# duxfrederic/lightcurver

Measured on AMD Instinct MI355X. Metric: cutouts/sec (PSF-fit + joint forward-model iter), 32x32 & 64x64 stamps, higher is better.
Workload: dtype f32

## Files before the change

### lightcurver_amd/csrc/psf_kernels.h

```cpp
#pragma once
#include <type_traits>
#include <utility>

#include "lc_common.h"
#include "starlet_device.h"

#ifndef LC_XPOLL_SLEEP
#define LC_XPOLL_SLEEP 2
#endif
#ifndef LC_P5_AHEAD
#define LC_P5_AHEAD 1
#endif
#ifndef LC_STARLET_LIVE_ADDR
#define LC_STARLET_LIVE_ADDR 1
#endif
#ifndef LC_SERIAL_TRIM
#define LC_SERIAL_TRIM 1
#endif
namespace lc {
constexpr int kXFlagStride = 16;

#ifdef LC_STAMPS
__device__ long long g_stamps[128];
#define LC_STAMP(k)                                                      \
  do {                                                                   \
    if ((blockIdx.x == 0 || blockIdx.x == 8) && threadIdx.x == 0 && it == A.n_iter - 1)  \
      g_stamps[(k) + (blockIdx.x == 8 ? 64 : 0)] = clock64();            \
  } while (0)
#else
#define LC_STAMP(k) do {} while (0)
#endif


struct PsfArgs {
  int F, S, n_iter, t0, hist_stride, mode;
  const float *data, *wgt;
  const float *W;
  const float *norms;
  const float *Tm;
  float *B, *mB, *sB;
  float *stars, *stars_m, *stars_s;
  float *hist;
  float *qscratch;
  float *out_loss, *out_chi2, *out_gstars, *out_ggrid, *out_gT, *out_model;
  float lam_sc, lam_hf;
  lc_adabelief_cfg ab;
  float *xch;
  int *xflags, *xabort;
  int launch_seq, heal, force_abort_it;
  const float *bkB, *bkmB, *bksB, *bkstars, *bkstars_m, *bkstars_s;
  int *heal_count;
  const float *ext_grad;
  const float *sched;
  float *B1, *mB1, *sB1;
  int xcd_fast;
};

typedef float lc_v4f __attribute__((ext_vector_type(4)));
__device__ __forceinline__ void store_sc1_x4(float *p, lc_v4f v) {
  asm volatile("global_store_dwordx4 %0, %1, off sc1\n\ts_nop 2" ::"v"(p), "v"(v) : "memory");
}
__device__ __forceinline__ void store_plain_x4(float *p, lc_v4f v) {
  asm volatile("global_store_dwordx4 %0, %1, off\n\ts_nop 2" ::"v"(p), "v"(v) : "memory");
}
__device__ __forceinline__ void store_sc1_f(float *p, float v) {
  asm volatile("global_store_dword %0, %1, off sc1" ::"v"(p), "v"(v) : "memory");
}
__device__ __forceinline__ void load_sc1_2x4(const float *p, lc_v4f &a, lc_v4f &b) {
  asm volatile("global_load_dwordx4 %0, %2, off sc1\n\tglobal_load_dwordx4 %1, %2, off offset:16 sc1\n\ts_waitcnt vmcnt(0)"
               : "=&v"(a), "=&v"(b)
               : "v"(p)
               : "memory");
}
__device__ __forceinline__ void load_sc1_2x4_1(const float *p, lc_v4f &a, lc_v4f &b, const float *ps, float &s) {
  asm volatile("global_load_dword %2, %4, off sc1\n\tglobal_load_dwordx4 %0, %3, off sc1\n\tglobal_load_dwordx4 %1, %3, off offset:16 sc1\n\ts_waitcnt vmcnt(0)"
               : "=&v"(a), "=&v"(b), "=&v"(s)
               : "v"(p), "v"(ps)
               : "memory");
}
__device__ __forceinline__ void load_sc1_x4(const float *p, lc_v4f &a) {
  asm volatile("global_load_dwordx4 %0, %1, off sc1\n\ts_waitcnt vmcnt(0)" : "=&v"(a) : "v"(p) : "memory");
}
__device__ __forceinline__ float load_sc1_f(const float *p) {
  float v;
  asm volatile("global_load_dword %0, %1, off sc1\n\ts_waitcnt vmcnt(0)" : "=&v"(v) : "v"(p) : "memory");
  return v;
}


template <int N_, int SS_, int PX_, int SG_, bool WC_ = false, int JB_ = 8>
struct PsfCfg {
  static constexpr int N = N_, SS = SS_, PX = PX_, SG = SG_;
  static constexpr bool WC = WC_;
  static constexpr int n = N / SS;
  static constexpr int NTHR = N * N / PX;
  static constexpr int NW = (NTHR + kWave - 1) / kWave;
  static constexpr int NT = ntaps(SS);
  static constexpr int J = ilog2(N);
  static constexpr int LR = 8;
  static constexpr int LC = (JB_ * (N_ / SS_) / 4 >= 64) ? 4 : 2;
  static constexpr int LA = LC;
  static constexpr int TS = N + 1;
  static constexpr int RS = n + 1;
  static constexpr int OFF_T = 0;
  static constexpr int SZ_T = WC_ ? N * (N + 2 * (N / 4 + 10) + 1) : N * TS;
  static constexpr int OFF_R = OFF_T + SZ_T;
  static constexpr int SZ_R2 = SG * n * TS;
  static constexpr int VS = WC_ ? n + 3 : RS, VO = WC_ ? 1 : 0;
  static constexpr int SZ_V = SG * N * VS;
  static constexpr int JB = JB_;
  static constexpr int AP = N / 4 + 10;
  static constexpr int TSA = N + 2 * AP + 1;
  static constexpr int APR = AP / SS + 2;
  static constexpr int JBP = JB + 1;
  static constexpr int WSZ = JB * TSA + (n + 2 * APR) * JBP;
  static constexpr int SZ_VR = (SZ_V > StarletLds<N>::FLOATS) ? SZ_V : StarletLds<N>::FLOATS;
  static constexpr int OFF_WSC = OFF_R + SZ_VR;
  static constexpr int SZ_R = WC ? (SZ_VR + NW * WSZ) : ((2 * SZ_R2 > SZ_V) ? 2 * SZ_R2 : SZ_V);
  static constexpr int OFF_RES = OFF_R + SZ_R;
  static constexpr int SZ_RES = WC ? 0 : SG * n * n;
  static constexpr int OFF_TAPS = OFF_RES + SZ_RES;
  static constexpr int NTP = NT + 3;
  static constexpr int SZ_TAPS = (16 * 4 * NTP + 1) / 2 * 2 + 16 * 2 * NT * 2;
  static constexpr int OFF_TAPP = OFF_TAPS + (16 * 4 * NTP + 1) / 2 * 2;
  static constexpr int OFF_RED = OFF_TAPS + SZ_TAPS;
  static constexpr int IPS = n * n / LC;
  static constexpr int IPS_PAD = (IPS + kWave - 1) / kWave * kWave;
  static constexpr int SLOTS = IPS_PAD / kWave;
  static constexpr int SZ_REDX = 16 * NW;
  static constexpr int SZ_RED = (WC ? 16 * (n / JB) * 5 : SG * SLOTS * 5) + SZ_REDX + NW + 8;
  static constexpr int OFF_REDX = OFF_RED + (WC ? 16 * (n / JB) * 5 : SG * SLOTS * 5);
  static constexpr int OFF_REDW = OFF_REDX + SZ_REDX;
  static constexpr int OFF_STAR = OFF_RED + SZ_RED;
  static constexpr int MAXS = 16;
  static constexpr int SZ_STAR = MAXS * 20 + 16;
  static constexpr int LDS_FLOATS = OFF_STAR + SZ_STAR;
  static_assert(WC || StarletLds<N>::FLOATS <= SZ_T + SZ_R + SZ_RES, "starlet ping-pong buffers must fit over T + R + RES");
  static_assert(PX % SS == 0 && N % PX == 0 && n % LR == 0 && n % LC == 0 && n % LA == 0 && n % JB == 0, "tiling");
  static_assert(LDS_FLOATS * 4 <= 163840, "LDS");
  static_assert(OFF_TAPP % 2 == 0, "tap pairs are read as 64-bit words");
  static_assert(NTHR <= 1024 && NTHR % kWave == 0, "threads");
  static_assert(!WC_ || PX_ <= 8, "the WC layout keeps the pixel state in registers");
};


template <int SS, int NT>
__device__ inline void tap_entry(float delta, int k, float &tap, float &dtap, int &bq) {
  const int o = (int)nearbyintf(delta);
  const int base = o - kRg - (SS - 1);
  int q = base / SS;
  if (q * SS > base) --q;
  bq = q;
  const int m = q * SS + k;
  const float inv_s2 = 1.0f / (kSigmaG * kSigmaG);
  const float nrm = 0.3989422804014327f / kSigmaG;
  float a = 0.f, d = 0.f;
#pragma unroll
  for (int dv = 0; dv < SS; ++dv) {
    const int t = m + dv;
    if (t >= o - kRg && t <= o + kRg) {
      const float x = (float)t - delta;
      const float p = nrm * expf(-0.5f * x * x * inv_s2);
      a += p;
      d += p * x * inv_s2;
    }
  }
  tap = a;
  dtap = d;
}

template <class C, bool SPLIT = false>
__global__ __launch_bounds__(C::NTHR) void psf_fit_kernel(PsfArgs A) {
  constexpr int N = C::N, SS = C::SS, PX = C::PX, SG = C::SG, n = C::n, NT = C::NT, J = C::J;
  constexpr int NTHR = C::NTHR, TS = C::TS, RS = C::RS, LR = C::LR, LC = C::LC, LA = C::LA;
  extern __shared__ __align__(16) float lds[];
  float *T = lds + C::OFF_T;
  float *R2t = lds + C::OFF_R;
  float *R2xt = R2t + C::SZ_R2;
  float *V = lds + C::OFF_R;
  float *RES = lds + C::OFF_RES;
  float *TAPS = lds + C::OFF_TAPS + 1;
  constexpr int NTP = C::NTP;
  lc_v2f *TAPP = (lc_v2f *)(lds + C::OFF_TAPP);
  float *REDX = lds + C::OFF_REDX;
  float *RED = lds + C::OFF_RED;
  float *REDW = lds + C::OFF_REDW;
  float *SCAL = REDW + C::NW;
  float *SP = lds + C::OFF_STAR;
  float *SGR = SP + C::MAXS * 4;
  float *SM = SGR + C::MAXS * 5;
  float *SV = SM + C::MAXS * 4;
  int *BQ = (int *)(SV + C::MAXS * 4);

  int f = blockIdx.x, role = 0;
  if constexpr (SPLIT) {
    f = ((int)blockIdx.x >> 4) * 8 + ((int)blockIdx.x & 7);
    role = ((int)blockIdx.x >> 3) & 1;
    if (f >= A.F) return;
  }
  const bool conv_role = !SPLIT || role == 0, starlet_role = !SPLIT || role == 1;
  const int my_xcc = SPLIT ? (int)(__builtin_amdgcn_s_getreg(20 | (3 << 11)) & 15u) : 0;
  int same_xcd = 0;
  const int tid0 = threadIdx.x;
  const int S = A.S;

  const float *dataf = A.data + (size_t)f * S * n * n;
  const float *wgtf = A.wgt + (size_t)f * S * n * n;

  if constexpr (!SPLIT) {
    if (A.heal) {
      if (__hip_atomic_load(A.xabort, __ATOMIC_RELAXED, __HIP_MEMORY_SCOPE_AGENT) != A.launch_seq) return;
      const size_t o = (size_t)f * N * N;
      for (int i = tid0; i < N * N; i += NTHR) {
        A.B[o + i] = A.bkB[o + i];
        A.mB[o + i] = A.bkmB[o + i];
        A.sB[o + i] = A.bksB[o + i];
      }
      if (tid0 < S * 4) {
        A.stars[(size_t)f * S * 4 + tid0] = A.bkstars[(size_t)f * S * 4 + tid0];
        A.stars_m[(size_t)f * S * 4 + tid0] = A.bkstars_m[(size_t)f * S * 4 + tid0];
        A.stars_s[(size_t)f * S * 4 + tid0] = A.bkstars_s[(size_t)f * S * 4 + tid0];
      }
      if (f == 0 && tid0 == 0) atomicAdd(A.heal_count, 1);
      __threadfence_block();
      __syncthreads();
    }
  }

  if constexpr (C::WC) {
    for (int i = tid0; i < C::SZ_T; i += NTHR) lds[C::OFF_T + i] = 0.f;
    for (int i = tid0; i < C::NW * C::WSZ; i += NTHR) lds[C::OFF_WSC + i] = 0.f;
  }
  if (tid0 < S * 4) {
    SP[tid0] = A.stars[(size_t)f * S * 4 + tid0];
    SM[tid0] = A.stars_m[(size_t)f * S * 4 + tid0];
    SV[tid0] = A.stars_s[(size_t)f * S * 4 + tid0];
  }
  __syncthreads();

  constexpr bool STATE_REGS = (PX <= 8);
  float *Bg = A.B, *mBg = A.mB, *sBg = A.sB;
  if constexpr (SPLIT && !STATE_REGS) {
    if (role == 1) {
      const size_t g0pix = (size_t)f * N * N + (size_t)(tid0 / (N / PX)) * N + (tid0 % (N / PX)) * PX;
#pragma unroll
      for (int q = 0; q < PX / 4; ++q) {
        ((float4 *)(A.B1 + g0pix))[q] = ((const float4 *)(A.B + g0pix))[q];
        ((float4 *)(A.mB1 + g0pix))[q] = ((const float4 *)(A.mB + g0pix))[q];
        ((float4 *)(A.sB1 + g0pix))[q] = ((const float4 *)(A.sB + g0pix))[q];
      }
      Bg = A.B1;
      mBg = A.mB1;
      sBg = A.sB1;
    }
  }
  float Bp[PX], Mp[PX], Sp_[PX], Tp[PX];
  {
    const size_t g0pix = (size_t)f * N * N + (size_t)(tid0 / (N / PX)) * N + (tid0 % (N / PX)) * PX;
#pragma unroll
    for (int q = 0; q < PX / 4; ++q) {
      if (STATE_REGS) {
        const float4 b = ((const float4 *)(A.B + g0pix))[q], t = ((const float4 *)(A.Tm + g0pix))[q];
        const float4 m = ((const float4 *)(A.mB + g0pix))[q], sv = ((const float4 *)(A.sB + g0pix))[q];
        Bp[4 * q] = b.x; Bp[4 * q + 1] = b.y; Bp[4 * q + 2] = b.z; Bp[4 * q + 3] = b.w;
        Tp[4 * q] = t.x; Tp[4 * q + 1] = t.y; Tp[4 * q + 2] = t.z; Tp[4 * q + 3] = t.w;
        Mp[4 * q] = m.x; Mp[4 * q + 1] = m.y; Mp[4 * q + 2] = m.z; Mp[4 * q + 3] = m.w;
        Sp_[4 * q] = sv.x; Sp_[4 * q + 1] = sv.y; Sp_[4 * q + 2] = sv.z; Sp_[4 * q + 3] = sv.w;
      }
    }
  }

  auto compute_taps = [&](int tid) {
    for (int e = tid; e < S * 2 * NTP; e += NTHR) {
      const int s = e / (2 * NTP), ax = (e / NTP) & 1, k = e % NTP - 1;
      float tap = 0.f, dtap = 0.f;
      int bq = 0;
      const float c_off = (N % 2 == 0) ? 0.5f : 0.0f;
      const float delta = fminf(fmaxf(SS * SP[s * 4 + 1 + ax], -(float)(N / 4)), (float)(N / 4)) + c_off;
      if (k >= 0 && k < NT) tap_entry<SS, NT>(delta, k, tap, dtap, bq);
      TAPS[(s * 4 + 2 * ax) * NTP + k] = tap;
      TAPS[(s * 4 + 2 * ax + 1) * NTP + k] = dtap;
      if (k >= 0 && k < NT) TAPP[(s * 2 + ax) * NT + k] = (lc_v2f){tap, dtap};
      if (k == 0) BQ[s * 2 + ax] = bq;
    }
  };
  auto step_stars = [&](int tid) {
#pragma clang fp contract(off)
    if (tid < S * 3) {
      const float lr = SCAL[0], bc1 = SCAL[1], bc2 = SCAL[2];
      const float b1 = A.ab.b1, b2 = A.ab.b2, eps = A.ab.eps, eps_root = A.ab.eps_root;
      const int s = tid / 3, q = tid % 3;
      const float g = SGR[s * 5 + 1 + q];
      const float mn = b1 * SM[s * 4 + q] + (1.f - b1) * g;
      const float dg = g - mn;
      const float sn = b2 * SV[s * 4 + q] + (1.f - b2) * dg * dg + eps_root;
      SM[s * 4 + q] = mn;
      SV[s * 4 + q] = sn;
      SP[s * 4 + q] -= lr * (mn * bc1) / (sqrtf(sn * bc2) + eps);
    }
  };
  auto update_stars_and_taps = [&](int tid) {
    step_stars(tid);
    __syncthreads();
    compute_taps(tid);
  };
  if (conv_role) compute_taps(tid0);
  constexpr bool TRIM = SPLIT && C::WC && PX == 8 && LC_SERIAL_TRIM;
  static_assert(!TRIM || 3 * C::MAXS <= kWave, "the x0 sums and the stars' step are lanes of one wave");
  [[maybe_unused]] float tpix_next[TRIM ? PX : 1];
  if constexpr (TRIM) {
    if (role == 0) {
      const int pu = tid0 / (N / PX), pv = (tid0 % (N / PX)) * PX;
#pragma unroll
      for (int p = 0; p < PX; ++p) {
        tpix_next[p] = Bp[p] + Tp[p];
        T[pu * C::TSA + C::AP + pv + p] = tpix_next[p];
      }
    }
    __syncthreads();
  }
  for (int it = 0; it < A.n_iter; ++it) {
    const int tglob = A.t0 + it;
    if constexpr (SPLIT) {
      if (A.force_abort_it == it && f == 0 && role == 1) {
        if (tid0 == 0) __hip_atomic_store(A.xabort, A.launch_seq, __ATOMIC_RELAXED, __HIP_MEMORY_SCOPE_AGENT);
        break;
      }
    }
    int tid = tid0;
    LC_LAUNDER(tid);
    const int lane = tid & 63, wid = tid >> 6;
    const int pu = tid / (N / PX);
    const int pv = (tid % (N / PX)) * PX;
    const size_t gpix = (size_t)f * N * N + (size_t)pu * N + pv;
    if (tid < 3 && A.mode == 1) SCAL[tid] = A.sched[3 * tglob + tid];
    LC_STAMP(0);
    float gB[PX];
#pragma unroll
    for (int p = 0; p < PX; ++p) gB[p] = 0.f;
    float tpix[PX];
    if (conv_role) {
    if constexpr (TRIM) {
#pragma unroll
      for (int p = 0; p < PX; ++p) tpix[p] = tpix_next[p];
    } else if (C::WC && STATE_REGS) {
#pragma unroll
      for (int p = 0; p < PX; ++p) {
        tpix[p] = Bp[p] + Tp[p];
        T[pu * C::TSA + C::AP + pv + p] = tpix[p];
      }
    } else if (STATE_REGS) {
#pragma unroll
      for (int p = 0; p < PX; ++p) T[pu * TS + pv + p] = Bp[p] + Tp[p];
    } else {
      const float4 *bp = (const float4 *)(Bg + gpix);
      const float4 *tp = (const float4 *)(A.Tm + gpix);
#pragma unroll
      for (int q = 0; q < PX / 4; ++q) {
        const float4 b = bp[q], t = tp[q];
        T[pu * TS + pv + 4 * q + 0] = b.x + t.x;
        T[pu * TS + pv + 4 * q + 1] = b.y + t.y;
        T[pu * TS + pv + 4 * q + 2] = b.z + t.z;
        T[pu * TS + pv + 4 * q + 3] = b.w + t.w;
      }
    }
    if (tid < S * 5) SGR[tid] = 0.f;

    for (int g0 = 0; g0 < S; g0 += SG) {
      if (!TRIM || g0 > 0) __syncthreads();
      LC_STAMP(1 + 5 * (g0 / SG));
      if constexpr (C::WC) {
        constexpr int JB = C::JB, NBLK = n / JB;
        float *wsc = lds + C::OFF_WSC + wid * C::WSZ;
        constexpr int TSA = C::TSA, AP = C::AP, APR = C::APR;
        float *R2w = wsc + AP, *RESw = wsc + JB * TSA + APR * C::JBP;
        int kdone = 0;
        for (int task = wid; task < SG * NBLK; task += C::NW, ++kdone) {
          progress_prio(kdone);
          const int sl = task / NBLK, blk = task % NBLK, s = g0 + sl;
          if (s >= S) continue;
          const int jd0 = blk * JB;
          const float *tx = TAPS + (s * 4 + 0) * NTP, *ty = tx + 2 * NTP, *dty = tx + 3 * NTP;
          const int bqx = BQ[s * 2 + 0], bqy = BQ[s * 2 + 1];
          const float amp = SP[s * 4 + 0], sky = SP[s * 4 + 3];
          constexpr int NI3 = (JB * (n / LC) + 63) / 64;
          float dpre[NI3][LC], wpre[NI3][LC];
#pragma unroll
          for (int i3 = 0; i3 < NI3; ++i3) {
            const int item = lane + 64 * i3;
            const bool ok = item < JB * (n / LC);
            const int jl = item % JB, a0 = (item / JB) * LC;
#pragma unroll
            for (int j = 0; j < LC; ++j) {
              const size_t pix = ok ? ((size_t)s * n * n + (size_t)(a0 + j) * n + jd0 + jl) : 0;
              const float dv = dataf[pix], wv = wgtf[pix];
              dpre[i3][j] = ok ? dv : 0.f;
              wpre[i3][j] = ok ? wv : 0.f;
            }
          }
          LC_STAMP(10);
          {
            const int ws = SS * (jd0 - bqx) - (NT - 1);
            if constexpr (SS == 2) {
              constexpr int NP = (NT + 1) / 2, WL2 = (JB - 1) + NP;
              lc_v2f tr2[NP];
#pragma unroll
              for (int h = 0; h < NP; ++h) tr2[h] = (lc_v2f){tx[NT - 1 - 2 * h], tx[NT - 2 - 2 * h]};
              for (int u = lane; u < N; u += 64) {
                lc_v2f win2[WL2];
                const float *trow = T + u * TSA + AP + ws;
#pragma unroll
                for (int i = 0; i < WL2; ++i) win2[i] = (lc_v2f){trow[2 * i], trow[2 * i + 1]};
                lc_v2f acc[JB];
#pragma unroll
                for (int j = 0; j < JB; ++j) acc[j] = (lc_v2f){0.f, 0.f};
#pragma unroll
                for (int h = 0; h < NP; ++h) {
#pragma unroll
                  for (int j = 0; j < JB; ++j) acc[j] = pk_fma(tr2[h], win2[j + h], acc[j]);
                }
#pragma unroll
                for (int j = 0; j < JB; ++j) R2w[j * TSA + u] = acc[j].x + acc[j].y;
              }
            } else {
              constexpr int WL = SS * (JB - 1) + NT;
              float tk[NT];
#pragma unroll
              for (int k = 0; k < NT; ++k) tk[k] = tx[k];
              for (int u = lane; u < N; u += 64) {
                float win[WL];
                const float *trow = T + u * TSA + AP + ws;
#pragma unroll
                for (int i = 0; i < WL; ++i) win[i] = trow[i];
#pragma unroll
                for (int j = 0; j < JB; ++j) {
                  float acc = 0.f;
#pragma unroll
                  for (int k = 0; k < NT; ++k) acc = fmaf(tk[k], win[SS * j - k + NT - 1], acc);
                  R2w[j * TSA + u] = acc;
                }
              }
            }
          }
          wave_lds_sync();
          LC_STAMP(11);
          float chi = 0.f, ga = 0.f, gy = 0.f, gs = 0.f;
          {
            constexpr int WL = SS * (LC - 1) + NT;
            lc_v2f tyd[NT];
#pragma unroll
            for (int k = 0; k < NT; ++k) tyd[k] = TAPP[(s * 2 + 1) * NT + k];
#pragma unroll
            for (int i3 = 0; i3 < NI3; ++i3) {
              const int item = lane + 64 * i3;
              if (item < JB * (n / LC)) {
                const int jl = item % JB, a0 = (item / JB) * LC;
                const int ws = SS * (a0 - bqy) - (NT - 1);
                float win[WL];
                const float *r2 = R2w + jl * TSA + ws;
#pragma unroll
                for (int i = 0; i < WL; ++i) win[i] = r2[i];
                float lgy = 0.f;
                lc_v2f fvys[LC];
#pragma unroll
                for (int j = 0; j < LC; ++j) fvys[j] = (lc_v2f){0.f, 0.f};
#pragma unroll
                for (int k = 0; k < NT; ++k) {
#pragma unroll
                  for (int j = 0; j < LC; ++j) fvys[j] = pk_fma(tyd[k], pk_bcast(win[SS * j - k + NT - 1]), fvys[j]);
                  if constexpr (LC == 4) asm volatile("" : "+v"(fvys[0]), "+v"(fvys[1]), "+v"(fvys[2]), "+v"(fvys[3]));
                  else asm volatile("" : "+v"(fvys[0]), "+v"(fvys[1]));
                }
#pragma unroll
                for (int j = 0; j < LC; ++j) {
                  const float fv = fvys[j].x, fy = fvys[j].y;
                  const float model = fmaf(amp, fv, sky);
                  const float res = model - dpre[i3][j];
                  const float rw = wpre[i3][j] * res;
                  chi = fmaf(rw, res, chi);
                  ga = fmaf(rw, fv, ga);
                  lgy = fmaf(rw, fy, lgy);
                  gs += rw;
                  RESw[(a0 + j) * C::JBP + jl] = rw;
                  if (A.out_model) A.out_model[(size_t)f * S * n * n + (size_t)s * n * n + (size_t)(a0 + j) * n + jd0 + jl] = model;
                }
                gy += lgy * amp * SS;
              }
            }
          }
          wave_sum4(chi, ga, gy, gs);
          if (lane == 0) {
            float *r = RED + (s * NBLK + blk) * 5;
            r[0] = chi;
            r[1] = ga;
            r[3] = gy;
            r[4] = gs;
          }
          wave_lds_sync();
          LC_STAMP(12);
          {
            constexpr int WI = (SS * LA - 1 + NT - 1) / SS + 1;
            constexpr int NI4 = (JB * (n / LA) + 63) / 64;
            if constexpr (SS == 2) {
              constexpr int NP = (NT + 1) / 2;
              lc_v2f py[NP];
#pragma unroll
              for (int q = 0; q < NP; ++q) py[q] = (lc_v2f){ty[2 * q], ty[2 * q - 1]};
#pragma unroll
              for (int i4 = 0; i4 < NI4; ++i4) {
                const int item = lane + 64 * i4;
                if (item < JB * (n / LA)) {
                  const int jl = item % JB, a0 = (item / JB) * LA;
                  lc_v2f out2[LA];
#pragma unroll
                  for (int h = 0; h < LA; ++h) out2[h] = (lc_v2f){0.f, 0.f};
                  const float *rcol = RESw + (bqy + a0) * C::JBP + jl;
#pragma unroll
                  for (int i = 0; i < WI; ++i) {
                    const lc_v2f rv = pk_bcast(rcol[i * C::JBP]);
#pragma unroll
                    for (int h = 0; h < LA; ++h)
                      if (i - h >= 0 && i - h < NP) out2[h] = pk_fma(py[i - h], rv, out2[h]);
                  }
                  float *vrow = V + (sl * N + SS * a0) * C::VS + C::VO + jd0 + jl;
#pragma unroll
                  for (int h = 0; h < LA; ++h) {
                    vrow[(2 * h) * C::VS] = out2[h].x;
                    vrow[(2 * h + 1) * C::VS] = out2[h].y;
                  }
                  if (jd0 + jl == 0) {
#pragma unroll
                    for (int r = 0; r < SS * LA; ++r) V[(sl * N + SS * a0 + r) * C::VS] = 0.f;
                  }
                  if (jd0 + jl == n - 1) {
#pragma unroll
                    for (int r = 0; r < SS * LA; ++r) V[(sl * N + SS * a0 + r) * C::VS + n + 1] = 0.f;
                  }
                }
              }
            } else {
              float tk[NT];
#pragma unroll
              for (int k = 0; k < NT; ++k) tk[k] = ty[k];
#pragma unroll
              for (int i4 = 0; i4 < NI4; ++i4) {
                const int item = lane + 64 * i4;
                if (item < JB * (n / LA)) {
                  const int jl = item % JB, a0 = (item / JB) * LA;
                  float out[SS * LA];
#pragma unroll
                  for (int r = 0; r < SS * LA; ++r) out[r] = 0.f;
                  const float *rcol = RESw + (bqy + a0) * C::JBP + jl;
#pragma unroll
                  for (int i = 0; i < WI; ++i) {
                    const float rv = rcol[i * C::JBP];
#pragma unroll
                    for (int k = 0; k < NT; ++k) {
                      const int rel = SS * i - k;
                      if (rel >= 0 && rel < SS * LA) out[rel] = fmaf(tk[k], rv, out[rel]);
                    }
                  }
#pragma unroll
                  for (int r = 0; r < SS * LA; ++r) V[(sl * N + SS * a0 + r) * C::VS + C::VO + jd0 + jl] = out[r];
                  if (jd0 + jl == 0) {
#pragma unroll
                    for (int r = 0; r < SS * LA; ++r) V[(sl * N + SS * a0 + r) * C::VS] = 0.f;
                  }
                  if (jd0 + jl == n - 1) {
#pragma unroll
                    for (int r = 0; r < SS * LA; ++r) V[(sl * N + SS * a0 + r) * C::VS + n + 1] = 0.f;
                  }
                }
              }
            }
          }
          wave_lds_sync();
          LC_STAMP(13);
        }
        __builtin_amdgcn_s_setprio(0);
        LC_STAMP(14);
#ifdef LC_STAMPS
        if (blockIdx.x == 0 && lane == 0 && it == A.n_iter - 1) g_stamps[20 + wid] = clock64();
#endif
        __syncthreads();
        LC_STAMP(15);
        if (tid < SG * 5) {
          const int sl = tid / 5, q = tid % 5;
          if (g0 + sl < S && q != 2) {
            float acc = 0.f;
            for (int k = 0; k < NBLK; ++k) acc += RED[((g0 + sl) * NBLK + k) * 5 + q];
            SGR[(g0 + sl) * 5 + q] = acc;
          }
        }
      } else {
      constexpr int NIT3 = (SG * C::IPS_PAD + NTHR - 1) / NTHR;
      float dpre[NIT3][LC], wpre[NIT3][LC];
#pragma unroll
      for (int i3 = 0; i3 < NIT3; ++i3) {
        const int item0 = wid * 64 + i3 * NTHR, item = item0 + lane;
        const int sl = item0 / C::IPS_PAD, within = item % C::IPS_PAD, s = g0 + sl;
        const bool ok = (item0 < SG * C::IPS_PAD) && (s < S) && (within < C::IPS);
        const int jd = within % n, a0 = (within / n) * LC;
#pragma unroll
        for (int j = 0; j < LC; ++j) {
          const size_t pix = ok ? ((size_t)s * n * n + (size_t)(a0 + j) * n + jd) : 0;
          const float dv = dataf[pix], wv = wgtf[pix];
          dpre[i3][j] = ok ? dv : 0.f;
          wpre[i3][j] = ok ? wv : 0.f;
        }
      }
      {
        constexpr int WL = SS * (LR - 1) + NT;
        constexpr int NSTRIP = n / LR;
        for (int item = tid; item < SG * N * NSTRIP; item += NTHR) {
          const int u = item % N, strip = (item / N) % NSTRIP, sl = item / (N * NSTRIP);
          if (g0 + sl >= S) continue;
          const float *tx = TAPS + ((g0 + sl) * 4 + 0) * NTP;
          const int bq = BQ[(g0 + sl) * 2 + 0];
          const int a0 = strip * LR;
          const int ws = SS * (a0 - bq) - (NT - 1);
          float win[WL];
#pragma unroll
          for (int i = 0; i < WL; ++i) {
            const int idx = ws + i;
            const int ci = min(max(idx, 0), N - 1);
            const float v = T[u * TS + ci];
            win[i] = (idx >= 0 && idx < N) ? v : 0.f;
          }
          float tk[NT];
#pragma unroll
          for (int k = 0; k < NT; ++k) tk[k] = tx[k];
#pragma unroll
          for (int j = 0; j < LR; ++j) {
            float acc = 0.f;
#pragma unroll
            for (int k = 0; k < NT; ++k) acc = fmaf(tk[k], win[SS * j - k + NT - 1], acc);
            R2t[(sl * n + a0 + j) * TS + u] = acc;
          }
        }
      }
      __syncthreads();
      LC_STAMP(2 + 5 * (g0 / SG));
      {
        constexpr int WL = SS * (LC - 1) + NT;
        constexpr int NSTRIP = n / LC;
#pragma unroll
        for (int i3 = 0; i3 < NIT3; ++i3) {
          const int item0 = wid * 64 + i3 * NTHR;
          if (item0 >= SG * C::IPS_PAD) break;
          const int item = item0 + lane;
          const int sl = item0 / C::IPS_PAD;
          const int within = item % C::IPS_PAD;
          const int s = g0 + sl;
          float chi = 0.f, ga = 0.f, gx = 0.f, gy = 0.f, gs = 0.f;
          if (s < S && within < C::IPS) {
            const int jd = within % n, strip = within / n;
            const float *ty = TAPS + (s * 4 + 2) * NTP, *dty = ty + NTP;
            const int bq = BQ[s * 2 + 1];
            const int a0 = strip * LC;
            const int ws = SS * (a0 - bq) - (NT - 1);
            const float amp = SP[s * 4 + 0], sky = SP[s * 4 + 3];
            float win[WL];
#pragma unroll
            for (int i = 0; i < WL; ++i) {
              const int idx = ws + i;
              const int ci = min(max(idx, 0), N - 1);
              const bool ok = (idx >= 0 && idx < N);
              const float v = R2t[(sl * n + jd) * TS + ci];
              win[i] = ok ? v : 0.f;
            }
            float tk[NT], dk[NT];
#pragma unroll
            for (int k = 0; k < NT; ++k) {
              tk[k] = ty[k];
              dk[k] = dty[k];
            }
#pragma unroll
            for (int j = 0; j < LC; ++j) {
              float fv = 0.f, fy = 0.f;
#pragma unroll
              for (int k = 0; k < NT; ++k) {
                const float w = win[SS * j - k + NT - 1];
                fv = fmaf(tk[k], w, fv);
                fy = fmaf(dk[k], w, fy);
              }
              const int id = a0 + j;
              const size_t pix = (size_t)s * n * n + (size_t)id * n + jd;
              const float d = dpre[i3][j], w = wpre[i3][j];
              const float model = fmaf(amp, fv, sky);
              const float res = model - d;
              const float rw = w * res;
              chi = fmaf(rw, res, chi);
              ga = fmaf(rw, fv, ga);
              gy = fmaf(rw, fy, gy);
              gs += rw;
              RES[(sl * n + id) * n + jd] = rw;
              if (A.out_model) A.out_model[(size_t)f * S * n * n + pix] = model;
            }
            gy *= amp * SS;
          }
          chi = wave_sum(chi);
          ga = wave_sum(ga);
          gx = wave_sum(gx);
          gy = wave_sum(gy);
          gs = wave_sum(gs);
          if (lane == 0) {
            float *r = RED + (sl * C::SLOTS + (item0 % C::IPS_PAD) / 64) * 5;
            r[0] = chi;
            r[1] = ga;
            r[2] = gx;
            r[3] = gy;
            r[4] = gs;
          }
        }
      }
      __syncthreads();
      LC_STAMP(3 + 5 * (g0 / SG));
      if (tid < SG * 5) {
        const int sl = tid / 5, q = tid % 5;
        if (g0 + sl < S && q != 2) {
          float acc = 0.f;
          for (int k = 0; k < C::SLOTS; ++k) acc += RED[(sl * C::SLOTS + k) * 5 + q];
          SGR[(g0 + sl) * 5 + q] = acc;
        }
      }
      {
        constexpr int WI = (SS * LA - 1 + NT - 1) / SS + 1;
        constexpr int NSTRIP = n / LA;
        for (int item = tid; item < SG * n * NSTRIP; item += NTHR) {
          const int jd = item % n, strip = (item / n) % NSTRIP, sl = item / (n * NSTRIP);
          if (g0 + sl >= S) continue;
          const float *ty = TAPS + ((g0 + sl) * 4 + 2) * NTP;
          const int bq = BQ[(g0 + sl) * 2 + 1];
          const int a0 = strip * LA;
          float tk[NT];
#pragma unroll
          for (int k = 0; k < NT; ++k) tk[k] = ty[k];
          float out[SS * LA];
#pragma unroll
          for (int r = 0; r < SS * LA; ++r) out[r] = 0.f;
#pragma unroll
          for (int i = 0; i < WI; ++i) {
            const int id = i + bq + a0;
            const int ci = min(max(id, 0), n - 1);
            float rv = RES[(sl * n + ci) * n + jd];
            rv = (id >= 0 && id < n) ? rv : 0.f;
#pragma unroll
            for (int k = 0; k < NT; ++k) {
              const int rel = SS * i - k;
              if (rel >= 0 && rel < SS * LA) out[rel] = fmaf(tk[k], rv, out[rel]);
            }
          }
#pragma unroll
          for (int r = 0; r < SS * LA; ++r) V[(sl * N + SS * a0 + r) * RS + jd] = out[r];
        }
      }
      __syncthreads();
      LC_STAMP(4 + 5 * (g0 / SG));
      }
      LC_STAMP(16);
      if constexpr (C::WC) {
        constexpr int WJ = (PX - 1 + NT - 1) / SS + 1;
        constexpr bool AHEAD = SPLIT && PX == 8 && LC_P5_AHEAD;
        if constexpr (AHEAD) {
          static_assert(SG % 8 == 0, "two stars per turn of the loop share a priority step");
          struct P5Ops {
            float vwin[WJ];
            lc_v2f txd[NT];
            float amp;
          };
          auto p5_star = [&](int sl, const P5Ops &use, auto on_the_way) {
            const int s = g0 + sl;
            lc_v2f accp[PX];
#pragma unroll
            for (int p = 0; p < PX; ++p) accp[p] = (lc_v2f){0.f, 0.f};
#pragma unroll
            for (int i = 0; i < WJ; ++i) {
              if (i == 4) on_the_way();
              const lc_v2f vv = pk_bcast(use.vwin[i]);
#pragma unroll
              for (int k = 0; k < NT; ++k) {
                const int rel = SS * i - k;
                if (rel >= 0 && rel < PX) accp[rel] = pk_fma(use.txd[k], vv, accp[rel]);
              }
            }
            float gxs = 0.f;
#pragma unroll
            for (int p = 0; p < PX; ++p) {
              gB[p] = fmaf(use.amp, accp[p].x, gB[p]);
              gxs = fmaf(accp[p].y, tpix[p], gxs);
            }
            gxs = wave_sum(gxs);
            if (lane == 0) REDX[s * C::NW + wid] = gxs;
          };
          auto nothing = [] {};
          auto p5_window = [&](int sl, P5Ops &o, int bq) {
            o.amp = SP[(g0 + sl) * 4 + 0];
            const float *vrow = V + (sl * N + pu) * C::VS + 1;
            const int jd0 = bq + pv / SS;
#pragma unroll
            for (int i = 0; i < WJ; ++i) o.vwin[i] = vrow[min(max(jd0 + i, -1), n)];
            __builtin_amdgcn_sched_barrier(0);
          };
          auto p5_taps = [&](int sl, P5Ops &o) {
            __builtin_amdgcn_sched_barrier(0);
#pragma unroll
            for (int k = 0; k < NT; ++k) o.txd[k] = TAPP[((g0 + sl) * 2 + 0) * NT + k];
            __builtin_amdgcn_sched_barrier(0);
          };
          const int ns = min(SG, S - g0);
          P5Ops opsA, opsB;
          int bqn = BQ[min(g0 + 1, S - 1) * 2 + 0];
          p5_window(0, opsA, BQ[g0 * 2 + 0]);
          p5_taps(0, opsA);
          int sl = 0;
#pragma clang loop unroll(disable)
          while (sl + 1 < ns) {
            progress_prio((4 * sl) / SG);
            const int bqnn = BQ[min(g0 + sl + 2, S - 1) * 2 + 0];
            p5_window(sl + 1, opsB, bqn);
            p5_star(sl, opsA, [&] { p5_taps(sl + 1, opsB); });
            if (sl + 2 >= ns) {
              opsA = opsB;
              sl += 1;
              break;
            }
            bqn = BQ[min(g0 + sl + 3, S - 1) * 2 + 0];
            p5_window(sl + 2, opsA, bqnn);
            p5_star(sl + 1, opsB, [&] { p5_taps(sl + 2, opsA); });
            sl += 2;
          }
          progress_prio((4 * sl) / SG);
          p5_star(sl, opsA, nothing);
        } else {
          for (int sl = 0; sl < SG; ++sl) {
            const int s = g0 + sl;
            if (s >= S) break;
            progress_prio((4 * sl) / SG);
            const int bq = BQ[s * 2 + 0];
            const float amp = SP[s * 4 + 0];
            lc_v2f txd[NT];
#pragma unroll
            for (int k = 0; k < NT; ++k) txd[k] = TAPP[(s * 2 + 0) * NT + k];
            lc_v2f accp[PX];
#pragma unroll
            for (int p = 0; p < PX; ++p) accp[p] = (lc_v2f){0.f, 0.f};
            const float *vrow = V + (sl * N + pu) * C::VS + 1;
            const int jd0 = bq + pv / SS;
            float vwin[WJ];
#pragma unroll
            for (int i = 0; i < WJ; ++i) vwin[i] = vrow[min(max(jd0 + i, -1), n)];
#pragma unroll
            for (int i = 0; i < WJ; ++i) {
              const lc_v2f vv = pk_bcast(vwin[i]);
#pragma unroll
              for (int k = 0; k < NT; ++k) {
                const int rel = SS * i - k;
                if (rel >= 0 && rel < PX) accp[rel] = pk_fma(txd[k], vv, accp[rel]);
              }
            }
            float gxs = 0.f;
#pragma unroll
            for (int p = 0; p < PX; ++p) {
              gB[p] = fmaf(amp, accp[p].x, gB[p]);
              gxs = fmaf(accp[p].y, tpix[p], gxs);
            }
            gxs = wave_sum(gxs);
            if (lane == 0) REDX[s * C::NW + wid] = gxs;
          }
        }
        __builtin_amdgcn_s_setprio(0);
      } else {
        constexpr int WJ = (PX - 1 + NT - 1) / SS + 1;
        for (int sl = 0; sl < SG; ++sl) {
          const int s = g0 + sl;
          if (s >= S) break;
          const float *tx = TAPS + (s * 4 + 0) * NTP, *dtx = tx + NTP;
          const int bq = BQ[s * 2 + 0];
          const float amp = SP[s * 4 + 0];
          float acc[PX], gxs = 0.f;
#pragma unroll
          for (int p = 0; p < PX; ++p) acc[p] = 0.f;
#pragma unroll
          for (int i = 0; i < WJ; ++i) {
            const int jd = i + bq + pv / SS;
            const int ci = min(max(jd, 0), n - 1);
            float vv = V[(sl * N + pu) * RS + ci];
            vv = (jd >= 0 && jd < n) ? vv : 0.f;
            float dsum = 0.f;
#pragma unroll
            for (int k = 0; k < NT; ++k) {
              const int rel = SS * i - k;
              if (rel >= 0 && rel < PX) {
                acc[rel] = fmaf(tx[k], vv, acc[rel]);
                dsum = fmaf(dtx[k], T[pu * TS + pv + rel], dsum);
              }
            }
            gxs = fmaf(vv, dsum, gxs);
          }
#pragma unroll
          for (int p = 0; p < PX; ++p) gB[p] = fmaf(amp, acc[p], gB[p]);
          gxs = wave_sum(gxs);
          if (lane == 0) REDX[s * C::NW + wid] = gxs;
        }
      }
      LC_STAMP(17);
    }
    if (A.ext_grad) {
#pragma unroll
      for (int p = 0; p < PX; ++p) gB[p] += A.ext_grad[gpix + p];
    }
    }
    if constexpr (TRIM) {
      if (role == 0) {
        LC_STAMP(41);
        float *mine = A.xch + (((size_t)f * 2 + (it & 1)) * 2 + 0) * (N * N + 64);
#pragma unroll
        for (int q = 0; q < PX / 4; ++q) {
          lc_v4f v;
          v.x = gB[4 * q];
          v.y = gB[4 * q + 1];
          v.z = gB[4 * q + 2];
          v.w = gB[4 * q + 3];
          if (same_xcd) store_plain_x4(mine + pu * N + pv + 4 * q, v);
          else store_sc1_x4(mine + pu * N + pv + 4 * q, v);
        }
        if (tid == 0 && it == 0) store_sc1_f(mine + N * N + 1, __int_as_float(my_xcc + 1));
      }
    }
    __syncthreads();
    LC_STAMP(40);
    {
      if (conv_role && tid < S) {
        float acc = 0.f;
#pragma unroll
        for (int w = 0; w < C::NW; ++w) acc += REDX[tid * C::NW + w];
        SGR[tid * 5 + 2] = acc * SP[tid * 4 + 0] * SS;
      }
    }

    if (A.out_gT) {
#pragma unroll
      for (int p = 0; p < PX; ++p) A.out_gT[gpix + p] = gB[p];
    }

    float l1 = 0.f;
    float z[PX];
#pragma unroll
    for (int p = 0; p < PX; ++p) z[p] = 0.f;
    if (starlet_role && (A.lam_sc != 0.f || A.lam_hf != 0.f)) {
      float bpix[PX];
      if (STATE_REGS) {
#pragma unroll
        for (int p = 0; p < PX; ++p) bpix[p] = Bp[p];
      } else {
        const float4 *bp = (const float4 *)(Bg + gpix);
#pragma unroll
        for (int q = 0; q < PX / 4; ++q) {
          const float4 b = bp[q];
          bpix[4 * q] = b.x;
          bpix[4 * q + 1] = b.y;
          bpix[4 * q + 2] = b.z;
          bpix[4 * q + 3] = b.w;
        }
      }
      constexpr bool LIVE_ADDR = SPLIT && STATE_REGS && LC_STARLET_LIVE_ADDR;
      starlet_l1_grad<N, PX, ilog2(N), LIVE_ADDR>(bpix, A.W ? A.W + (size_t)f * J * N * N : nullptr, A.norms,
                                                  A.qscratch + (size_t)f * J * N * N, A.lam_sc, A.lam_hf,
                                                  C::WC ? lds + C::OFF_R : lds, tid, l1, z);
    }
    LC_STAMP(42);
    if (!TRIM || role == 1) {
      {
        const float wl = wave_sum(l1);
        if (lane == 0) REDW[wid] = wl;
      }
      __syncthreads();
    }
    float tl1 = 0.f;
    if (tid == 0 && starlet_role)
      for (int w = 0; w < C::NW; ++w) tl1 += REDW[w];
    LC_STAMP(44);
    if constexpr (SPLIT) {
      constexpr int XS = N * N + 64;
      float *mine = A.xch + (((size_t)f * 2 + (it & 1)) * 2 + role) * XS;
      const float *theirs = A.xch + (((size_t)f * 2 + (it & 1)) * 2 + (1 - role)) * XS;
      const int poff = pu * N + pv;
      if (!TRIM || role == 1) {
#pragma unroll
      for (int q = 0; q < PX / 4; ++q) {
        lc_v4f v;
        v.x = role ? z[4 * q] : gB[4 * q];
        v.y = role ? z[4 * q + 1] : gB[4 * q + 1];
        v.z = role ? z[4 * q + 2] : gB[4 * q + 2];
        v.w = role ? z[4 * q + 3] : gB[4 * q + 3];
        if (same_xcd) store_plain_x4(mine + poff + 4 * q, v);
        else store_sc1_x4(mine + poff + 4 * q, v);
      }
      if (tid == 0 && role == 1) {
        if (same_xcd) asm volatile("global_store_dword %0, %1, off" ::"v"(mine + N * N), "v"(tl1) : "memory");
        else store_sc1_f(mine + N * N, tl1);
      }
      if (tid == 0 && it == 0) store_sc1_f(mine + N * N + 1, __int_as_float(my_xcc + 1));
      }
      constexpr bool TAPS_LATE = STATE_REGS;
      if (role == 0 && A.mode == 1) {
        if constexpr (TRIM) wave_lds_sync();
        if (TAPS_LATE) step_stars(tid);
        else update_stars_and_taps(tid);
      }
      asm volatile("s_waitcnt vmcnt(0)" ::: "memory");
      __syncthreads();
      LC_STAMP(45);
      int *OK = (int *)(SCAL + 5);
      if (tid == 0) {
        if (same_xcd) asm volatile("global_store_dword %0, %1, off" ::"v"(A.xflags + ((size_t)f * 2 + role) * kXFlagStride), "v"(it + 1) : "memory");
        else __hip_atomic_store(A.xflags + ((size_t)f * 2 + role) * kXFlagStride, it + 1, __ATOMIC_RELAXED, __HIP_MEMORY_SCOPE_AGENT);
        int ok = 1, spins = 0;
        while (__hip_atomic_load(A.xflags + ((size_t)f * 2 + (1 - role)) * kXFlagStride, __ATOMIC_RELAXED, __HIP_MEMORY_SCOPE_AGENT) < it + 1) {
          __builtin_amdgcn_s_sleep(LC_XPOLL_SLEEP);
          ++spins;
          if (spins > (1 << 21) ||
              ((spins & 255) == 0 && __hip_atomic_load(A.xabort, __ATOMIC_RELAXED, __HIP_MEMORY_SCOPE_AGENT) == A.launch_seq)) {
            __hip_atomic_store(A.xabort, A.launch_seq, __ATOMIC_RELAXED, __HIP_MEMORY_SCOPE_AGENT);
            ok = 0;
            break;
          }
        }
        if (it == 0 && ok) OK[1] = (A.xcd_fast && __float_as_int(load_sc1_f(theirs + N * N + 1)) == my_xcc + 1) ? 1 : 0;
        *OK = ok;
#ifdef LC_XCH_ACQUIRE
        __builtin_amdgcn_fence(__ATOMIC_ACQUIRE, "agent");
        asm volatile("s_waitcnt vmcnt(0)" ::: "memory");
#endif
      }
      if (TAPS_LATE && role == 0 && A.mode == 1) compute_taps((tid + NTHR / 2) % NTHR);
      __syncthreads();
      LC_STAMP(46);
      if (*OK == 0) break;
      if (it == 0) same_xcd = OK[1];
      float other[PX];
      float tl1_other = 0.f;
      if constexpr (PX == 8) {
        lc_v4f a, b;
        load_sc1_2x4_1(theirs + poff, a, b, theirs + N * N, tl1_other);
        other[0] = a.x; other[1] = a.y; other[2] = a.z; other[3] = a.w;
        other[4] = b.x; other[5] = b.y; other[6] = b.z; other[7] = b.w;
      } else {
#pragma unroll
        for (int q = 0; q < PX / 4; ++q) {
          lc_v4f a;
          load_sc1_x4(theirs + poff + 4 * q, a);
          other[4 * q] = a.x; other[4 * q + 1] = a.y; other[4 * q + 2] = a.z; other[4 * q + 3] = a.w;
        }
      }
#pragma unroll
      for (int p = 0; p < PX; ++p) {
        if (role) gB[p] = other[p]; else z[p] = other[p];
      }
      if (tid == 0 && role == 0) tl1 = (PX == 8) ? tl1_other : load_sc1_f(theirs + N * N);
      LC_STAMP(47);
    }
    if (!TRIM && tid == 0 && conv_role) {
      float chi = 0.f;
      for (int s = 0; s < S; ++s) chi += SGR[s * 5];
      const float loss = 0.5f * chi + tl1;
      A.hist[(size_t)f * A.hist_stride + tglob] = loss;
      if (A.out_loss) A.out_loss[f] = loss;
      if (A.out_chi2) A.out_chi2[f] = chi;
    }
    if (A.out_ggrid) {
#pragma unroll
      for (int p = 0; p < PX; ++p) A.out_ggrid[gpix + p] = gB[p] + z[p];
    }
    if (A.out_gstars && tid < S * 4) {
      const int s = tid / 4, q = tid % 4;
      A.out_gstars[(size_t)f * S * 4 + tid] = SGR[s * 5 + 1 + q];
    }
    if (A.mode == 1) {
#pragma clang fp contract(off)
      const float lr = SCAL[0], bc1 = SCAL[1], bc2 = SCAL[2];
      const float b1 = A.ab.b1, b2 = A.ab.b2, eps = A.ab.eps, eps_root = A.ab.eps_root;
      if (STATE_REGS) {
#pragma unroll
        for (int p = 0; p < PX; ++p) {
          const float g = gB[p] + z[p];
          const float mn = b1 * Mp[p] + (1.f - b1) * g;
          const float dg = g - mn;
          const float sn = b2 * Sp_[p] + (1.f - b2) * dg * dg + eps_root;
          Mp[p] = mn;
          Sp_[p] = sn;
          Bp[p] -= lr * (mn * bc1) * __builtin_amdgcn_rcpf(__builtin_amdgcn_sqrtf(sn * bc2) + eps);
        }
      }
      if constexpr (!STATE_REGS) {
        float4 *bp = (float4 *)(Bg + gpix);
        float4 *mp = (float4 *)(mBg + gpix);
        float4 *sp = (float4 *)(sBg + gpix);
        float4 bq[PX / 4], mq[PX / 4], sq[PX / 4];
#pragma unroll
        for (int q = 0; q < PX / 4; ++q) {
          bq[q] = bp[q];
          mq[q] = mp[q];
          sq[q] = sp[q];
        }
#pragma unroll
        for (int q = 0; q < PX / 4; ++q) {
          float *bb = &bq[q].x, *mm = &mq[q].x, *ss_ = &sq[q].x;
#pragma unroll
          for (int e = 0; e < 4; ++e) {
            const float g = gB[4 * q + e] + z[4 * q + e];
            const float mn = b1 * mm[e] + (1.f - b1) * g;
            const float dg = g - mn;
            const float sn = b2 * ss_[e] + (1.f - b2) * dg * dg + eps_root;
            mm[e] = mn;
            ss_[e] = sn;
            bb[e] -= lr * (mn * bc1) * __builtin_amdgcn_rcpf(__builtin_amdgcn_sqrtf(sn * bc2) + eps);
          }
        }
#pragma unroll
        for (int q = 0; q < PX / 4; ++q) {
          bp[q] = bq[q];
          mp[q] = mq[q];
          sp[q] = sq[q];
        }
      }
      if constexpr (!SPLIT) update_stars_and_taps(tid);
    }
    if constexpr (TRIM) {
      if (role == 0) {
#pragma unroll
        for (int p = 0; p < PX; ++p) {
          tpix_next[p] = Bp[p] + Tp[p];
          T[pu * C::TSA + C::AP + pv + p] = tpix_next[p];
        }
        if (tid == 0) {
          float chi = 0.f;
          for (int s = 0; s < S; ++s) chi += SGR[s * 5];
          const float loss = 0.5f * chi + tl1;
          A.hist[(size_t)f * A.hist_stride + tglob] = loss;
          if (A.out_loss) A.out_loss[f] = loss;
          if (A.out_chi2) A.out_chi2[f] = chi;
        }
      }
    }
    __syncthreads();
    LC_STAMP(43);
  }

  if (A.mode == 1 && STATE_REGS && conv_role) {
    const size_t g0pix = (size_t)f * N * N + (size_t)(tid0 / (N / PX)) * N + (tid0 % (N / PX)) * PX;
#pragma unroll
    for (int q = 0; q < PX / 4; ++q) {
      ((float4 *)(A.B + g0pix))[q] = make_float4(Bp[4 * q], Bp[4 * q + 1], Bp[4 * q + 2], Bp[4 * q + 3]);
      ((float4 *)(A.mB + g0pix))[q] = make_float4(Mp[4 * q], Mp[4 * q + 1], Mp[4 * q + 2], Mp[4 * q + 3]);
      ((float4 *)(A.sB + g0pix))[q] = make_float4(Sp_[4 * q], Sp_[4 * q + 1], Sp_[4 * q + 2], Sp_[4 * q + 3]);
    }
  }
  if (A.mode == 1 && tid0 < S * 4 && conv_role) {
    A.stars[(size_t)f * S * 4 + tid0] = SP[tid0];
    A.stars_m[(size_t)f * S * 4 + tid0] = SM[tid0];
    A.stars_s[(size_t)f * S * 4 + tid0] = SV[tid0];
  }
}

}
```

Before: 60.27 million.

## Software-pipeline per-wave conv tasks by prefetching next task's pixels and rows

Adds a task-ahead path for the split, WC, PX==8 configuration. Each wave now issues the global pixel/weight loads and the row-convolution inputs for its next task while it finishes the column pass of the current one, with a sched_barrier to keep the loads early. The zeroing of V's border columns also moves out of the per-task loop into a single pass at kernel start. This aims to hide global-load latency and drop repeated border stores, at the cost of more live registers, a strict shape static_assert, and a duplicated code path.

Result: faster. 63.29 million (median of 6 runs) (+5.0%).

```diff
diff --git a/lightcurver_amd/csrc/psf_kernels.h b/lightcurver_amd/csrc/psf_kernels.h
--- a/lightcurver_amd/csrc/psf_kernels.h
+++ b/lightcurver_amd/csrc/psf_kernels.h
@@ -16,6 +16,12 @@
 #endif
 #ifndef LC_SERIAL_TRIM
 #define LC_SERIAL_TRIM 1
+#endif
+#ifndef LC_TASK_AHEAD
+#define LC_TASK_AHEAD 1
+#endif
+#ifndef LC_V_ZERO_ONCE
+#define LC_V_ZERO_ONCE LC_TASK_AHEAD
 #endif
 namespace lc {
 constexpr int kXFlagStride = 16;
@@ -308,6 +314,16 @@
   constexpr bool TRIM = SPLIT && C::WC && PX == 8 && LC_SERIAL_TRIM;
   static_assert(!TRIM || 3 * C::MAXS <= kWave, "the x0 sums and the stars' step are lanes of one wave");
   [[maybe_unused]] float tpix_next[TRIM ? PX : 1];
+  constexpr bool C2_SPLIT = SPLIT && C::WC && PX == 8;
+  constexpr bool TASK_AHEAD = C2_SPLIT && LC_TASK_AHEAD, V_ZERO_ONCE = C2_SPLIT && LC_V_ZERO_ONCE;
+  if constexpr (V_ZERO_ONCE) {
+    if (role == 0) {
+      for (int i = tid0; i < SG * N; i += NTHR) {
+        V[i * C::VS] = 0.f;
+        V[i * C::VS + n + 1] = 0.f;
+      }
+    }
+  }
   if constexpr (TRIM) {
     if (role == 0) {
       const int pu = tid0 / (N / PX), pv = (tid0 % (N / PX)) * PX;
@@ -374,6 +390,165 @@
         float *wsc = lds + C::OFF_WSC + wid * C::WSZ;
         constexpr int TSA = C::TSA, AP = C::AP, APR = C::APR;
         float *R2w = wsc + AP, *RESw = wsc + JB * TSA + APR * C::JBP;
+        if constexpr (TASK_AHEAD) {
+          static_assert(SS == 2 && N == kWave && JB * (n / LC) == kWave && LA == LC, "one item per lane in each pass of a task");
+          constexpr int NP = (NT + 1) / 2, WL2 = (JB - 1) + NP, WL = SS * (LC - 1) + NT, WI = (SS * LA - 1 + NT - 1) / SS + 1;
+          const int jl = lane % JB, a0 = (lane / JB) * LC;
+          const int ntask = min(SG, S - g0) * NBLK;
+          float dpre[LC], wpre[LC];
+          lc_v2f tr2[NP], win2[WL2];
+          lc_v2f py[NP];
+          float rv[WI];
+          auto pixel_request = [&](int task) {
+            const int s = g0 + task / NBLK, jd0 = (task % NBLK) * JB;
+#pragma unroll
+            for (int j = 0; j < LC; ++j) {
+              const size_t pix = (size_t)s * n * n + (size_t)(a0 + j) * n + jd0 + jl;
+              dpre[j] = dataf[pix];
+              wpre[j] = wgtf[pix];
+            }
+          };
+          auto row_request = [&](int task, int bqx) {
+            const int s = g0 + task / NBLK, jd0 = (task % NBLK) * JB;
+            const float *tx = TAPS + (s * 4 + 0) * NTP;
+#pragma unroll
+            for (int h = 0; h < NP; ++h) tr2[h] = (lc_v2f){tx[NT - 1 - 2 * h], tx[NT - 2 - 2 * h]};
+            const float *trow = T + lane * TSA + AP + SS * (jd0 - bqx) - (NT - 1);
+#pragma unroll
+            for (int i = 0; i < WL2; ++i) win2[i] = (lc_v2f){trow[2 * i], trow[2 * i + 1]};
+          };
+          auto row_fma_store = [&] {
+            lc_v2f acc[JB];
+#pragma unroll
+            for (int j = 0; j < JB; ++j) acc[j] = (lc_v2f){0.f, 0.f};
+#pragma unroll
+            for (int h = 0; h < NP; ++h) {
+#pragma unroll
+              for (int j = 0; j < JB; ++j) acc[j] = pk_fma(tr2[h], win2[j + h], acc[j]);
+            }
+#pragma unroll
+            for (int j = 0; j < JB; ++j) R2w[j * TSA + lane] = acc[j].x + acc[j].y;
+          };
+          auto tcol_request = [&](int task, int bqy) {
+            const float *ty = TAPS + ((g0 + task / NBLK) * 4 + 2) * NTP;
+#pragma unroll
+            for (int q = 0; q < NP; ++q) py[q] = (lc_v2f){ty[2 * q], ty[2 * q - 1]};
+            const float *rcol = RESw + (bqy + a0) * C::JBP + jl;
+#pragma unroll
+            for (int i = 0; i < WI; ++i) rv[i] = rcol[i * C::JBP];
+          };
+          auto tcol_fma_store = [&](int task) {
+            const int sl = task / NBLK, jd0 = (task % NBLK) * JB;
+            lc_v2f out2[LA];
+#pragma unroll
+            for (int h = 0; h < LA; ++h) out2[h] = (lc_v2f){0.f, 0.f};
+#pragma unroll
+            for (int i = 0; i < WI; ++i) {
+              const lc_v2f rr = pk_bcast(rv[i]);
+#pragma unroll
+              for (int h = 0; h < LA; ++h)
+                if (i - h >= 0 && i - h < NP) out2[h] = pk_fma(py[i - h], rr, out2[h]);
+            }
+            float *vrow = V + (sl * N + SS * a0) * C::VS + C::VO + jd0 + jl;
+#pragma unroll
+            for (int h = 0; h < LA; ++h) {
+              vrow[(2 * h) * C::VS] = out2[h].x;
+              vrow[(2 * h + 1) * C::VS] = out2[h].y;
+            }
+            if constexpr (!V_ZERO_ONCE) {
+              if (jd0 + jl == 0) {
+#pragma unroll
+                for (int r = 0; r < SS * LA; ++r) V[(sl * N + SS * a0 + r) * C::VS] = 0.f;
+              }
+              if (jd0 + jl == n - 1) {
+#pragma unroll
+                for (int r = 0; r < SS * LA; ++r) V[(sl * N + SS * a0 + r) * C::VS + n + 1] = 0.f;
+              }
+            }
+          };
+          int task = __builtin_amdgcn_readfirstlane(wid), kdone = 0;
+          int bqy = 0;
+          if (task < ntask) {
+            progress_prio(0);
+            pixel_request(task);
+            LC_STAMP(10);
+            row_request(task, BQ[(g0 + task / NBLK) * 2 + 0]);
+            bqy = BQ[(g0 + task / NBLK) * 2 + 1];
+            row_fma_store();
+            wave_lds_sync();
+          }
+#pragma clang loop unroll(disable)
+          for (; task < ntask; task += C::NW, ++kdone) {
+            progress_prio(kdone);
+            LC_STAMP(11);
+            const int sl = task / NBLK, blk = task % NBLK, s = g0 + sl, jd0 = blk * JB;
+            const bool more = task + C::NW < ntask;
+            const int snext = min(g0 + (task + C::NW) / NBLK, S - 1);
+            const int bqx_next = BQ[snext * 2 + 0], bqy_next = BQ[snext * 2 + 1];
+            const float amp = SP[s * 4 + 0], sky = SP[s * 4 + 3];
+            float chi = 0.f, ga = 0.f, gy = 0.f, gs = 0.f;
+            {
+              lc_v2f tyd[NT];
+#pragma unroll
+              for (int k = 0; k < NT; ++k) tyd[k] = TAPP[(s * 2 + 1) * NT + k];
+              float win[WL];
+              const float *r2 = R2w + jl * TSA + SS * (a0 - bqy) - (NT - 1);
+#pragma unroll
+              for (int i = 0; i < WL; ++i) win[i] = r2[i];
+              float lgy = 0.f;
+              lc_v2f fvys[LC];
+#pragma unroll
+              for (int j = 0; j < LC; ++j) fvys[j] = (lc_v2f){0.f, 0.f};
+#pragma unroll
+              for (int k = 0; k < NT; ++k) {
+#pragma unroll
+                for (int j = 0; j < LC; ++j) fvys[j] = pk_fma(tyd[k], pk_bcast(win[SS * j - k + NT - 1]), fvys[j]);
+                asm volatile("" : "+v"(fvys[0]), "+v"(fvys[1]), "+v"(fvys[2]), "+v"(fvys[3]));
+              }
+#pragma unroll
+              for (int j = 0; j < LC; ++j) {
+                const float fv = fvys[j].x, fy = fvys[j].y;
+                const float model = fmaf(amp, fv, sky);
+                const float res = model - dpre[j];
+                const float rw = wpre[j] * res;
+                chi = fmaf(rw, res, chi);
+                ga = fmaf(rw, fv, ga);
+                lgy = fmaf(rw, fy, lgy);
+                gs += rw;
+                RESw[(a0 + j) * C::JBP + jl] = rw;
+                if (A.out_model) A.out_model[(size_t)f * S * n * n + (size_t)s * n * n + (size_t)(a0 + j) * n + jd0 + jl] = model;
+              }
+              gy += lgy * amp * SS;
+            }
+            wave_sum4(chi, ga, gy, gs);
+            if (lane == 0) {
+              float *r = RED + (s * NBLK + blk) * 5;
+              r[0] = chi;
+              r[1] = ga;
+              r[3] = gy;
+              r[4] = gs;
+            }
+            wave_lds_sync();
+            LC_STAMP(12);
+            if (more) {
+              LC_STAMP(19);
+              pixel_request(task + C::NW);
+              row_request(task + C::NW, bqx_next);
+              tcol_request(task, bqy);
+              __builtin_amdgcn_sched_barrier(0);
+              row_fma_store();
+              tcol_fma_store(task);
+              wave_lds_sync();
+              LC_STAMP(18);
+            } else {
+              tcol_request(task, bqy);
+              tcol_fma_store(task);
+              wave_lds_sync();
+              LC_STAMP(13);
+            }
+            bqy = bqy_next;
+          }
+        } else {
         int kdone = 0;
         for (int task = wid; task < SG * NBLK; task += C::NW, ++kdone) {
           progress_prio(kdone);
@@ -528,13 +703,15 @@
                     vrow[(2 * h) * C::VS] = out2[h].x;
                     vrow[(2 * h + 1) * C::VS] = out2[h].y;
                   }
-                  if (jd0 + jl == 0) {
-#pragma unroll
-                    for (int r = 0; r < SS * LA; ++r) V[(sl * N + SS * a0 + r) * C::VS] = 0.f;
-                  }
-                  if (jd0 + jl == n - 1) {
-#pragma unroll
-                    for (int r = 0; r < SS * LA; ++r) V[(sl * N + SS * a0 + r) * C::VS + n + 1] = 0.f;
+                  if constexpr (!V_ZERO_ONCE) {
+                    if (jd0 + jl == 0) {
+#pragma unroll
+                      for (int r = 0; r < SS * LA; ++r) V[(sl * N + SS * a0 + r) * C::VS] = 0.f;
+                    }
+                    if (jd0 + jl == n - 1) {
+#pragma unroll
+                      for (int r = 0; r < SS * LA; ++r) V[(sl * N + SS * a0 + r) * C::VS + n + 1] = 0.f;
+                    }
                   }
                 }
               }
@@ -576,6 +753,7 @@
           }
           wave_lds_sync();
           LC_STAMP(13);
+        }
         }
         __builtin_amdgcn_s_setprio(0);
         LC_STAMP(14);
```
